# lucidrains/transfusion-pytorch

Hardware: AMD Instinct MI355X
Metric: train samples/sec, dim512 d8 seq1024 text+latent (higher is better)
Workload: dtype bf16; 1 GPU; BASELINE config 2: Transfusion dim=512 depth=8 heads=8 dim_head=64 num_text_tokens=256 dim_latent=384; per-GPU batch 64 x seq 1024 (32 x [24 text tokens + (4,384) latent] per sample); step = pack + fwd + bwd + clip(0.5) + Adam(3e-4) (one GPU: no gradient exchange); global_batch=64, seq_len=1024, parallelism=dp1

## Files before the change

include/tfx.h:

```cpp
#ifndef TFX_H
#define TFX_H
#include <stdint.h>
#ifdef __cplusplus
extern "C" {
#endif

#ifndef TFX_BF16_DEFINED
typedef uint16_t tfx_bf16;
#endif

enum { TFX_EPI_BF16 = 0, TFX_EPI_F32 = 1, TFX_EPI_SILU = 2, TFX_EPI_RESID = 3, TFX_EPI_GEGLU = 4, TFX_EPI_GEGLU_BWD = 5, TFX_EPI_QKV_NORM_ROPE = 6 };

typedef struct {
  const tfx_bf16* A; int32_t lda;
  const tfx_bf16* A2; int32_t lda2; int32_t K1;
  const tfx_bf16* B; int32_t ldb;
  int32_t M, N, K;
  int32_t epi;
  void* C; int32_t ldc;
  void* C2; int32_t ldc2;
  const float* bias;
  const tfx_bf16* R; int32_t ldr; int32_t resid_mapped;
  const int32_t* rowmap;
  const int32_t* a_rowmap;
  const tfx_bf16* aux; int32_t ldaux;
  int32_t qk_heads;
  const float* qk_gamma_q; const float* qk_gamma_k;
  const int32_t* qk_rot_pos; const float* qk_cos; const float* qk_sin;
  float qk_q_scale, qk_norm_scale;
  float* qk_plan; float qk_softcap;
  tfx_bf16* qk_cache; int32_t qk_ld_cache; const int32_t* qk_cache_pos;
  const void* prefetch; int64_t prefetch_bytes;
} tfx_gemm_nt_args;
int tfx_gemm_nt(const tfx_gemm_nt_args* a, void* stream);
int tfx_gemm_nt_plan(const tfx_gemm_nt_args* a, int32_t* kind, int32_t* grid);

int tfx_mfma_peak_probe(const void* ops, float* out, int32_t iters, int32_t blocks, void* stream);

typedef struct {
  const tfx_bf16* A; int32_t lda; int32_t a_cols;
  const tfx_bf16* B; int32_t ldb; int32_t b_cols;
  int32_t M, N, K;
  float* C; int32_t ldc;
  const int32_t* rowmap;
  int32_t k_valid;
  int32_t splits;
  int32_t accumulate;
  float alpha;
  const int32_t* a_rowmap;
  const int32_t* b_rowmap;
  float* colsum;
  int32_t k_group;
  const void* group_next;
} tfx_gemm_tn_args;
int tfx_gemm_tn(const tfx_gemm_tn_args* a, void* stream);
int tfx_gemm_tn_plan(const tfx_gemm_tn_args* a, int32_t* kind, int32_t* tiles, int32_t* splits, int32_t* grid);

typedef struct {
  const tfx_bf16 *q, *k, *v; int32_t ld_q, ld_k, ld_v;
  const tfx_bf16* gate; int32_t ld_gate;
  const int32_t* kv_end;
  const int32_t* q_start;
  tfx_bf16* out; int32_t ld_out;
  float* lse;
  int32_t b, h, n;
  float softcap;
  int32_t n_kv;
  const tfx_bf16* dout; int32_t ld_dout;
  tfx_bf16* do_eff; int32_t ld_do;
  float* delta;
  tfx_bf16* dgate; int32_t ld_dgate;
  tfx_bf16 *dq, *dk, *dv; int32_t ld_dq, ld_dk, ld_dv;
  int32_t order;
  const float* sc_plan;
  const int32_t* q_row0; const int32_t* q_cnt;
  const tfx_bf16* nr_qkv; int32_t nr_ld_qkv;
  tfx_bf16* nr_dqkv; int32_t nr_ld_dqkv;
  const float* nr_gamma_q; const float* nr_gamma_k;
  const int32_t* nr_rot_pos; const float* nr_cos; const float* nr_sin;
  float nr_q_scale, nr_norm_scale;
  float* nr_dgamma_q; float* nr_dgamma_k;
  int32_t laser;
} tfx_attn_args;
int tfx_attn_fwd(const tfx_attn_args* a, void* stream);
int tfx_attn_bwd(const tfx_attn_args* a, void* stream);

int tfx_decode_attn(const tfx_attn_args* a, void* stream);

typedef struct {
  int32_t T, H;
  const tfx_bf16* v; int32_t ld_v;
  tfx_bf16* vl; int32_t ld_vl;
  const int32_t* rowmap;
  float c;
// ... 278 lines not shown
```

transfusion_pytorch_amd/csrc/attention.hip:

```cpp
#include "tfx_kernels.h"
#include "attn_asm_clobbers.inc"

namespace tfx {

constexpr int DH = 64;
constexpr int LDT = 72;

struct TileRegs { u32x4 r[2]; };
TFX_DEV void tile_gload(TileRegs& tr, const bf16* base, int ld, int row0, int nrows) {
#pragma unroll
  for (int i = 0; i < 2; i++) {
    int c = threadIdx.x + 256 * i;
    int row = min(row0 + (c >> 3), nrows - 1);
    tr.r[i] = *(const u32x4*)(base + (size_t)row * ld + (c & 7) * 8);
  }
}
TFX_DEV void tile_sstore(const TileRegs& tr, bf16* lds) {
#pragma unroll
  for (int i = 0; i < 2; i++) {
    int c = threadIdx.x + 256 * i;
    *(u32x4*)(lds + (c >> 3) * LDT + (c & 7) * 8) = tr.r[i];
  }
}
TFX_DEV bf16x8 lds_rowfrag(const bf16* lds, int r0, int ks) {
// ... 482 lines not shown
  if (vid >= T * p.h) return;
  const unsigned t = vid / (unsigned)p.h; const int h = (int)(vid - t * p.h);
  const bf16x8 d8 = *(const bf16x8*)(p.dout + (size_t)t * p.ld_dout + h * DH + sub * 8);
  const bf16x8 o8 = *(const bf16x8*)(p.out + (size_t)t * p.ld_out + h * DH + sub * 8);
  const float g = sigmoidf_(bf2f(p.gate[(size_t)t * p.ld_gate + h]));
  if (p.laser) {
    const float rg = __builtin_amdgcn_rcpf(fmaxf(g, 1e-30f));
    float dg = 0.f, ds = 0.f; bf16x8 e8;
#pragma unroll
    for (int e = 0; e < 8; e++) {
      const float d = bf2f(d8[e]), og = bf2f(o8[e]);
      dg += d * og; ds += d;
      e8[e] = f2bf(d * g * __expf(-og * rg));
    }
    *(bf16x8*)(p.do_eff + (size_t)t * p.ld_do + h * DH + sub * 8) = e8;
    dg = group8_sum(dg); ds = group8_sum(ds);
    if (sub == 0) {
      const unsigned bb = t / (unsigned)p.n, i = t - bb * p.n;
      p.delta[((size_t)bb * p.h + h) * p.n + i] = ds * g;
      p.dgate[(size_t)t * p.ld_dgate + h] = f2bf(dg * (1.f - g));
    }
    return;
  }
  float dl = 0.f; bf16x8 e8;
#pragma unroll
  for (int e = 0; e < 8; e++) { float d = bf2f(d8[e]); dl += d * bf2f(o8[e]); e8[e] = f2bf(d * g); }
  *(bf16x8*)(p.do_eff + (size_t)t * p.ld_do + h * DH + sub * 8) = e8;
  dl = group8_sum(dl);
  if (sub == 0) {
    const unsigned bb = t / (unsigned)p.n, i = t - bb * p.n;
    p.delta[((size_t)bb * p.h + h) * p.n + i] = dl;
    p.dgate[(size_t)t * p.ld_dgate + h] = f2bf(dl * (1.f - g));
  }
}

__global__ __launch_bounds__(256, 2) void attn_bwd_dq_kernel(tfx_attn_args p) {
  __shared__ __attribute__((aligned(16))) bf16 Ks[64 * LDT];
  __shared__ __attribute__((aligned(16))) bf16 Vs[64 * LDT];
  const int l = threadIdx.x & 63, w = threadIdx.x >> 6, hi = l >> 5;
  const int n = p.n;
  const BlockId bi = decode_block(p.order, (n + 127) / 128, true);
  const int h = bi.h, b = bi.b, q0 = bi.tile * 128;
  const size_t tok0 = (size_t)b * n;
  const bf16* qb = p.q + tok0 * p.ld_q + h * DH;
  const bf16* kb_ = p.k + tok0 * p.ld_k + h * DH;
  const bf16* vb = p.v + tok0 * p.ld_v + h * DH;
  const bf16* dob = p.do_eff + tok0 * p.ld_do + h * DH;
  const int qrow = q0 + w * 32 + (l & 31);
  const int qc = min(qrow, n - 1);
  const int kve = p.kv_end[tok0 + qc];
  const int kv_limit = p.kv_end[tok0 + min(q0 + 127, n - 1)];
  const int nt = (kv_limit + 63) / 64;
  const float lse2 = p.lse[((size_t)b * p.h + h) * n + qc] * LOG2E;
  float dlt;
  const int kve_min = wave_min_i(kve);
// ... 464 lines not shown
      for (int e = 0; e < 8; e++) pg[e] = 0.f;
      wave_block_store_nr<1>(st, kv, p, tok0 + k0 + w * 32, (p.h + h) * DH, rows, pg);
      wave_block_store(st, vv, p.dv + (tok0 + k0 + w * 32) * p.ld_dv + h * DH, p.ld_dv, rows);
      nr_flush_dgamma(pg, sg, p.nr_dgamma_k);
    } else {
      wave_block_store(st, kv, p.dk + (tok0 + k0 + w * 32) * p.ld_dk + h * DH, p.ld_dk, rows);
      wave_block_store(st, vv, p.dv + (tok0 + k0 + w * 32) * p.ld_dv + h * DH, p.ld_dv, rows);
    }
  }
}

static dim3 attn_grid(const tfx_attn_args& q) { return dim3(q.h, q.b, (q.n + 127) / 128); }
int attn_fwd(const tfx_attn_args& p, hipStream_t s) {
  if (p.n <= 0 || p.b <= 0 || p.h <= 0) return -1;
  if ((p.ld_q | p.ld_k | p.ld_v | p.ld_out) & 7) return -2;
  if (!(p.softcap > 0.f) || p.softcap * LOG2E > 96.f) return -3;
  tfx_attn_args q = p; q.order = 1;
  static int use_asm = -1;
  if (use_asm < 0) { const char* e = getenv("TFX_ATTN_ASM"); use_asm = (e && e[0] == '1') ? 1 : 0; }
  if (use_asm && p.n_kv == 0 && !p.q_cnt && !p.q_row0 && p.sc_plan) hipLaunchKernelGGL(attn_fwd_pipe_kernel<true>, attn_grid(q), dim3(256), 0, s, q);
  else hipLaunchKernelGGL(attn_fwd_pipe_kernel<false>, attn_grid(q), dim3(256), 0, s, q);
  return (int)hipGetLastError();
}
int attn_bwd(const tfx_attn_args& p, hipStream_t s) {
  if (p.n <= 0 || p.b <= 0 || p.h <= 0) return -1;
  if ((p.ld_q | p.ld_k | p.ld_v | p.ld_out | p.ld_dout | p.ld_do | p.ld_dq | p.ld_dk | p.ld_dv) & 7) return -2;
  if (!(p.softcap > 0.f) || p.softcap * LOG2E > 96.f) return -3;
  long long nthreads = (long long)p.b * p.n * p.h * 8;
  if (nthreads >= (1ll << 31)) return -4;
  if (p.nr_qkv) {
    if (!p.nr_dqkv || !p.nr_gamma_q || !p.nr_gamma_k || !p.nr_rot_pos || !p.nr_cos || !p.nr_sin || !p.nr_dgamma_q || !p.nr_dgamma_k) return -5;
    if (((p.nr_ld_qkv | p.nr_ld_dqkv) & 7) || (((uintptr_t)p.nr_qkv | (uintptr_t)p.nr_dqkv) & 15)) return -5;
  }
  tfx_attn_args q = p; q.order = 1;
  static int pipe = -1;
  if (pipe < 0) { const char* e = getenv("TFX_ATTN_BWD_PIPE"); pipe = (e && e[0] == '0') ? 0 : 1; }
  hipLaunchKernelGGL(attn_bwd_prep_kernel, dim3((unsigned)((nthreads + 255) / 256)), dim3(256), 0, s, q);
  hipLaunchKernelGGL(attn_bwd_dkv_kernel, attn_grid(q), dim3(256), 0, s, q);
  if (pipe) hipLaunchKernelGGL(attn_bwd_dq_pipe_kernel, attn_grid(q), dim3(256), 0, s, q);
  else hipLaunchKernelGGL(attn_bwd_dq_kernel, attn_grid(q), dim3(256), 0, s, q);
  return (int)hipGetLastError();
}

}
```

transfusion_pytorch_amd/csrc/gemm.hip:

```cpp
#include "tfx_common.h"
#include "tfx_kernels.h"
#include <type_traits>
#include <cmath>
#include <cstring>
#include <vector>
#include <algorithm>
#include <mutex>

namespace tfx {

constexpr int BM = 128, BN = 128, BK = 64;

template <int EPI> struct Epilogue;

TFX_DEV void store_bf16x4(bf16* dst, f32x4 v) {
  bf16x4 o; o[0] = f2bf(v[0]); o[1] = f2bf(v[1]); o[2] = f2bf(v[2]); o[3] = f2bf(v[3]);
  *(bf16x4*)dst = o;
}

TFX_DEV f32x4 add_bias(const GemmNT& p, int n, f32x4 v) {
  if (p.bias) { f32x4 b = *(const f32x4*)(p.bias + n); v += b; }
  return v;
}

// ... 275 lines not shown
    }
    if (i + 1 < NI) load_r(i + 1);
    bf16* s = st + (i & 1) * 2048;
#pragma unroll
    for (int j = 0; j < 2; j++)
#pragma unroll
      for (int g = 0; g < 4; g++) {
        const int col = j * 32 + 8 * g + 4 * hi;
        const bf16x4 rv = *(const bf16x4*)(sr + r * 64 + (((col >> 3) ^ ((r >> 1) & 7)) << 3) + (col & 7));
        f32x4 v;
#pragma unroll
        for (int e = 0; e < 4; e++) v[e] = acc[i][j][4 * g + e] + bias[j][g][e] + bf2f(rv[e]);
        stage_put4(s, r, col, v);
      }
    bf16x8 v[4];
#pragma unroll
    for (int q = 0; q < 4; q++) {
      const int row = q * 8 + (l >> 3);
      v[q] = *(const bf16x8*)(s + row * 64 + ((ch ^ ((row >> 1) & 7)) << 3));
    }
#pragma unroll
    for (int q = 0; q < 4; q++)
      if (col_ok && mo[i][q] >= 0) *(bf16x8*)((bf16*)p.C + (size_t)mo[i][q] * p.ldc + n_w + ch * 8) = v[q];
  }
}
TFX_DEV void stage_put4_32(bf16* st, int row, int col, f32x4 v) {
  bf16x4 o; o[0] = f2bf(v[0]); o[1] = f2bf(v[1]); o[2] = f2bf(v[2]); o[3] = f2bf(v[3]);
  *(bf16x4*)(st + row * 32 + (((col >> 3) ^ ((row >> 2) & 3)) << 3) + (col & 7)) = o;
}
constexpr int GTAB_N = 4096;
TFX_DEV float gelu_grid(const float* gtab, float g) {
  const float x = g * 128.f;
  const float xr = __builtin_amdgcn_fmed3f(__builtin_rintf(x), -1024.f, 1023.f);
  const float d = x - xr;
  const f32x4 c = *(const f32x4*)(gtab + 4 * ((int)xr + 1024));
  return fmaf(fmaf(c[2], d, c[1]), d, c[0]);
}
TFX_DEV GegluUVH geglu_uvh_grid(const float* gtab, float a, float g) {
  const float x = g * 128.f;
  const float xr = __builtin_amdgcn_fmed3f(__builtin_rintf(x), -1024.f, 1023.f);
  const float d = x - xr;
  const f32x4 c = *(const f32x4*)(gtab + 4 * ((int)xr + 1024));
  const float t = fmaf(c[2], d, c[1]);
  GegluUVH r; r.u = fmaf(t, d, c[0]);
  r.h = a * r.u;
  r.v = (a * 128.f) * fmaf(c[2], d, t);
// ... 283 lines not shown
  }
}
template <int EPI> TFX_DEV bool can_stage(const GemmNT& p) {
  bool ok = ((p.ldc | p.N) & 7) == 0 && (((uintptr_t)p.C) & 15) == 0;
  if constexpr (EPI == EPI_GEGLU) ok = ok && (p.ldc2 & 7) == 0 && (((uintptr_t)p.C2) & 15) == 0;
  if constexpr (EPI == EPI_GEGLU_BWD) ok = ok && (p.ldaux & 7) == 0 && (((uintptr_t)p.aux) & 15) == 0 && p.N >= 64;
  if constexpr (EPI == EPI_RESID) ok = ok && (p.ldr & 7) == 0 && (((uintptr_t)p.R) & 15) == 0 && p.N >= 8;
  return ok;
}
template <int EPI, int NI>
TFX_DEV void nt_epilogue(const GemmNT& p, f32x16 (&acc)[NI][2], int m_w, int n_w, bf16* st, const float* gtab = nullptr, bool use_tab = false, int lane = -1) {
  if constexpr (EPI == EPI_BF16) {
    if (can_stage<EPI>(p)) {
      if (!p.rowmap && !p.bias) staged_epilogue_bf16<NI, true>(p, acc, m_w, n_w, st, lane);
      else staged_epilogue_bf16<NI, false>(p, acc, m_w, n_w, st, lane);
      return;
    }
  } else if constexpr (EPI == EPI_F32) {
    if (((p.ldc | p.N) & 3) == 0 && (((uintptr_t)p.C) & 15) == 0) { staged_epilogue_f32<NI>(p, acc, m_w, n_w, st); return; }
  } else if constexpr (EPI == EPI_GEGLU || EPI == EPI_GEGLU_BWD) {
    if (can_stage<EPI>(p)) { staged_epilogue_geglu<EPI, NI>(p, acc, m_w, n_w, st, gtab, use_tab); return; }
  } else if constexpr (EPI == EPI_RESID) {
    if (can_stage<EPI>(p)) { staged_epilogue_resid<NI>(p, acc, m_w, n_w, st); return; }
  }
  if constexpr (EPI == EPI_QKNR) staged_epilogue_qknr<NI>(p, acc, m_w, n_w, st);
  else fast_epilogue<EPI, NI>(p, acc, m_w, n_w, lane);
}


template <int EPI>
__global__ __launch_bounds__(256, 2) void gemm_nt_kernel(GemmNT p) {
  extern __shared__ __attribute__((aligned(16))) char smem_raw[];
  bf16* As = (bf16*)smem_raw;
  bf16* Bs = As + 2 * BM * BK;

  const int t = threadIdx.x, l = t & 63, w = t >> 6;
  const int wm = w >> 1, wn = w & 1, hi = l >> 5;
  const int ntn = (p.N + BN - 1) / BN;
  const int bid = xcd_remap(blockIdx.x, gridDim.x);
  const int m0 = (bid / ntn) * BM, n0 = (bid % ntn) * BN;
  const int nk = p.K / BK;

  int srow[4], skc[4];
  const bf16 *ga[4], *ga2[4], *gb[4];
#pragma unroll
  for (int i = 0; i < 4; i++) {
// ... 658 lines not shown
    const int k0 = kt * BK;
    const bool second = p.A2 && k0 >= p.K1;
    glds16_asm(second ? gA2[h][j] + (k0 - p.K1) : gA[h][j] + k0, lds + ((kt & 1) * 4 + h) * HALF + (w * 16 + j * 8) * BK);
  };
  auto issueB1 = [&](int kt, int h, int j) { glds16_asm(gB[h][j] + kt * BK, lds + ((kt & 1) * 4 + 2 + h) * HALF + (w * 16 + j * 8) * BK); };
  const int ra = wr * 64 + (l & 31), rb = wc * 32 + (l & 31);
  auto ldA = [&](int kt, int h, int il, int ks) {
    const int r = ra + il * 32;
    return *(const bf16x8*)(lds + ((kt & 1) * 4 + h) * HALF + r * BK + (((ks * 2 + hi) ^ ((r >> 1) & 7)) << 3));
  };
  auto ldB = [&](int kt, int h, int ks) {
    return *(const bf16x8*)(lds + ((kt & 1) * 4 + 2 + h) * HALF + rb * BK + (((ks * 2 + hi) ^ ((rb >> 1) & 7)) << 3));
  };

  f32x16 acc[4][2];
#pragma unroll
  for (int i = 0; i < 4; i++)
#pragma unroll
    for (int j = 0; j < 2; j++)
#pragma unroll
      for (int r = 0; r < 16; r++) acc[i][j][r] = 0.f;

#ifdef TFX_PP_TIMING
  unsigned long long* stamps = (unsigned long long*)(EPI == EPI_GEGLU_BWD ? (const void*)p.R : (const void*)p.aux) + (size_t)blockIdx.x * 8;
#define PP_STAMP(i) { if (t == 0) stamps[i] = __builtin_readcyclecounter(); }
#else
#define PP_STAMP(i)
#endif
  PP_STAMP(0)
  asm volatile("s_waitcnt vmcnt(0)" ::: "memory");
  if constexpr (EPI == EPI_QKNR) {
    if (p.qk_plan && blockIdx.x == 0 && w == 0) softcap_plan_write(p.qk_gamma_q, p.qk_gamma_k, p.qk_norm_scale, p.qk_q_scale, p.qk_softcap, p.qk_plan);
  }
  const float* gtab_lds = (const float*)(smem_raw + 8 * HALF * 2);
  if constexpr (EPI == EPI_GEGLU) {
    if (gtab) {
#pragma unroll
      for (int j = 0; j < 4; j++) glds16_asm((const bf16*)gtab + (size_t)(w * 4 + j) * 512 + l * 8, (const bf16*)gtab_lds + (w * 4 + j) * 512);
    }
  }
  issueA(0, 0); issueB(0, 0); issueA(0, 1); issueB(0, 1);
  if (nk > 1) {
    issueA(1, 0); issueB(1, 0);
    asm volatile("s_waitcnt vmcnt(4)" ::: "memory");
  } else {
    asm volatile("s_waitcnt vmcnt(0)" ::: "memory");
  }
// ... 587 lines not shown
    auto phi = [](double g) { return 0.39894228040143267794 * exp(-0.5 * g * g); };
    const double st = 1.0 / 128.0;
    for (int i = 0; i < 2048; i++) {
      const double g = (i - 1024) * st;
      h[4 * i] = (float)(g * Phi(g));
      h[4 * i + 1] = (float)((Phi(g) + g * phi(g)) * st);
      h[4 * i + 2] = (float)(0.5 * phi(g) * (2.0 - g * g) * st * st);
      h[4 * i + 3] = 0.f;
    }
    float* d = nullptr;
    if (hipMalloc(&d, h.size() * 4) == hipSuccess && hipMemcpy(d, h.data(), h.size() * 4, hipMemcpyHostToDevice) == hipSuccess) tab[dev] = d;
  }
  return tab[dev];
}
struct NtPlan { int kind, grid; };
static bool nt_ow_takes(const GemmNT& p);
static bool nt_owp_takes(const GemmNT& p);
static NtPlan nt_plan(const GemmNT& p) {
  const int grid = ((p.M + BM - 1) / BM) * ((p.N + BN - 1) / BN);
  const int t256 = ((p.M + BM2 - 1) / BM2) * ((p.N + BN2 - 1) / BN2);
  const bool dma = use_glds() && (p.N & 3) == 0;
  const int grid_sd = ((p.M + 63) / 64) * ((p.N + 63) / 64);
  const int grid_sk = ((p.M + SK_BM - 1) / SK_BM) * ((p.N + SK_BN - 1) / SK_BN);
  if (dma && p.M <= 1024 && p.K % SD_BK == 0 && p.K >= 8 * SD_BK && grid_sd <= 256) return {NT_DECODE, grid_sd};
  if (dma && (p.M <= 512 || (p.M <= 1024 && grid_sk <= 256))) return {NT_SKINNY, grid_sk};
  static int pp_min = -1;
  if (pp_min < 0) { const char* e = getenv("TFX_NT_PP_MIN"); pp_min = e ? atoi(e) : 512; }
  if (dma && t256 >= pp_min) return {!nt_ow_takes(p) ? NT_PP : nt_owp_takes(p) ? NT_OWP : NT_OW, t256};
  if (dma && grid <= 256 && p.K >= 4 * BK) return {NT_MID, grid};
  return {dma ? NT_GLDS : NT_FALLBACK, grid};
}

constexpr int PP_STAGGER = 12000;
template <int EPI> static void launch_pp(const GemmNT& p, int grid, hipStream_t s) {
  static uint32_t attr_pp = 0;
  const float* gtab = EPI == EPI_GEGLU ? gelu_table() : nullptr;
  const int smem2 = 2 * (BM2 * BK + BN2 * BK) * 2 + (gtab ? GTAB_N * 8 : 0);
  ensure_smem_attr((const void*)gemm_nt_pp_kernel<EPI>, 2 * (BM2 * BK + BN2 * BK) * 2 + GTAB_N * 8, attr_pp);
  hipLaunchKernelGGL(gemm_nt_pp_kernel<EPI>, dim3(grid), dim3(512), smem2, s, p, PP_STAGGER, gtab);
}
static int nt_ow_mode() {
  static int ow = -1;
  if (ow < 0) { const char* e = getenv("TFX_NT_OW"); ow = e ? atoi(e) : 1; }
  return ow;
}
static bool nt_ow_takes(const GemmNT& p) {
  const int ow = nt_ow_mode();
  if (ow == 0 || p.a_rowmap || p.A2) return false;
  if (!(p.epi == EPI_BF16 || (p.epi == EPI_F32 && p.K >= 1024))) return false;
  if ((((uintptr_t)p.A | (uintptr_t)p.B) & 15) != 0) return false;
// ... 73 lines not shown
  return !p.rowmap && !p.a_rowmap && !p.bias && ((p.ldc | p.ldc2 | p.N) & 7) == 0 && (((uintptr_t)p.C | (uintptr_t)p.C2) & 15) == 0 && 2 * hd <= p.N && p.ldc2 >= 2 * hd;
}
static int gemm_nt_qknr(const GemmNT& p, hipStream_t s) {
  if (p.qk_heads <= 0 || !p.C2 || !p.qk_gamma_q || !p.qk_gamma_k || !p.qk_rot_pos || !p.qk_cos || !p.qk_sin) return -5;
  if (qknr_fusable(p)) {
    const NtPlan pl = nt_plan(p);
    if (pl.kind == NT_PP) { launch_pp<EPI_QKNR>(p, pl.grid, s); return (int)hipGetLastError(); }
    static uint32_t attr_sd = 0;
    const int smem_sd = 4 * SD_ST * SD_SLOT * 2;
    ensure_smem_attr((const void*)gemm_nt_decode_kernel<EPI_QKNR>, smem_sd, attr_sd);
    hipLaunchKernelGGL(gemm_nt_decode_kernel<EPI_QKNR>, dim3(pl.grid + prefetch_blocks(p)), dim3(256), smem_sd, s, p, pl.grid);
    return (int)hipGetLastError();
  }
  GemmNT q = p; q.epi = EPI_BF16; q.C2 = nullptr;
  const int rc = launch_nt<EPI_BF16>(q, s);
  if (rc) return rc;
  tfx_qk_norm_rope_args a;
  memset(&a, 0, sizeof(a));
  a.T = p.M; a.H = p.qk_heads; a.qkv = (const tfx_bf16*)p.C; a.ld_qkv = p.ldc; a.qk = (tfx_bf16*)p.C2; a.ld_qk = p.ldc2;
  a.gamma_q = p.qk_gamma_q; a.gamma_k = p.qk_gamma_k; a.rot_pos = p.qk_rot_pos; a.cos_tab = p.qk_cos; a.sin_tab = p.qk_sin;
  a.q_scale = p.qk_q_scale; a.norm_scale = p.qk_norm_scale; a.sc_plan = p.qk_plan; a.softcap = p.qk_softcap;
  a.cache = p.qk_cache; a.ld_cache = p.qk_ld_cache; a.cache_pos = p.qk_cache_pos;
  return tfx_qk_norm_rope_fwd(&a, (void*)s);
}

int gemm_nt(const GemmNT& p, hipStream_t s) {
  if (p.K % BK != 0 || (p.A2 && p.K1 % BK != 0) || p.M <= 0 || p.N <= 0) return -1;
  if ((p.lda | p.ldb) & 7) return -2;
  switch (p.epi) {
    case EPI_BF16: return launch_nt<EPI_BF16>(p, s);
    case EPI_F32: return launch_nt<EPI_F32>(p, s);
    case EPI_SILU: return launch_nt<EPI_SILU>(p, s);
    case EPI_RESID: return launch_nt<EPI_RESID>(p, s);
    case EPI_GEGLU: return (p.N % 64) ? -3 : launch_nt<EPI_GEGLU>(p, s);
    case EPI_GEGLU_BWD: return (p.N % 64) ? -3 : launch_nt<EPI_GEGLU_BWD>(p, s);
    case EPI_QKNR: return gemm_nt_qknr(p, s);
  }
  return -4;
}

template <bool SUM, int FA, int FB, int WN, int WK, int NST> static void launch_tn_wide(const GemmTN& q, int grid, hipStream_t s) {
  constexpr int smem = NST * (FA * WN + FB * WK) / 4 * MW_ROWS * 128 * 2;
  static uint32_t attr = 0;
  ensure_smem_attr((const void*)gemm_tn_wide_kernel<SUM, FA, FB, WN, WK, NST>, smem, attr);
  hipLaunchKernelGGL((gemm_tn_wide_kernel<SUM, FA, FB, WN, WK, NST>), dim3(grid), dim3(64 * WN * WK), smem, s, q);
}

struct TnPlan { int kind, tiles, splits, grid; };
static int tn_ow_mode();
static bool tn_ow_operands_ok(const GemmTN& q);
static TnPlan tn_plan(const GemmTN& q) {
#ifdef TFX_TN_TIMING
  const bool dma_ok = true;
#else
  const bool dma_ok = use_glds() && q.M % TN_BMK == 0 && !q.a_rowmap && !q.b_rowmap && q.a_cols >= 8 && q.b_cols >= 8;
#endif
  const int t44 = ((q.N + 255) / 256) * ((q.K + 255) / 256), t22 = ((q.N + 127) / 128) * ((q.K + 127) / 128);
  TnPlan pl;
  pl.kind = !dma_ok ? -1 : (t44 >= 8 ? 2 : 0);
// ... 129 lines not shown
```

transfusion_pytorch_amd/csrc/tfx_common.h:

```cpp
#pragma once
#include <hip/hip_runtime.h>
#include <stdint.h>
#include <mutex>

typedef __bf16 bf16;
typedef __attribute__((ext_vector_type(8))) __bf16 bf16x8;
typedef __attribute__((ext_vector_type(4))) __bf16 bf16x4;
typedef __attribute__((ext_vector_type(2))) __bf16 bf16x2;
typedef __attribute__((ext_vector_type(16))) float f32x16;
typedef __attribute__((ext_vector_type(4))) float f32x4;
typedef __attribute__((ext_vector_type(2))) float f32x2_t;
typedef __attribute__((ext_vector_type(4))) short s16x4;
typedef __attribute__((ext_vector_type(4))) uint32_t u32x4;
typedef __attribute__((ext_vector_type(2))) uint32_t u32x2;

#define TFX_DEV __device__ __forceinline__

TFX_DEV float bf2f(bf16 v) { return (float)v; }
TFX_DEV bf16 f2bf(float v) { return (bf16)v; }

#ifndef TFX_BPERMUTE_REDUCE
#define TFX_DPP_STEP(OP, V, CTRL, ROWMASK, IDENT)                                                                     \
  V = OP(V, __builtin_bit_cast(float, __builtin_amdgcn_update_dpp(__builtin_bit_cast(int, (float)(IDENT)),            \
                                                                    __builtin_bit_cast(int, V), CTRL, ROWMASK, 0xf, false)))
// ... 102 lines not shown
  asm volatile("s_mov_b32 m0, %1\n\ts_nop 0\n\tglobal_load_lds_dwordx4 %0, off" ::"v"(g), "s"(lds_addr) : "memory");
}

TFX_DEV float gelu_cdf(float g, float& E) {
  E = __expf(-0.5f * g * g);
  const float t = __builtin_amdgcn_rcpf(fmaf(0.3275911f * 0.70710678118654752440f, fabsf(g), 1.f));
  const float poly = t * fmaf(t, fmaf(t, fmaf(t, fmaf(t, 1.061405429f, -1.453152027f), 1.421413741f), -0.284496736f), 0.254829592f);
  const float half_erf = 0.5f - 0.5f * poly * E;
  return 0.5f + __builtin_copysignf(half_erf, g);
}
TFX_DEV float gelu_erf(float x) { float E; return x * gelu_cdf(x, E); }
struct GegluUVH { float u, v, h; };
TFX_DEV GegluUVH geglu_uvh(float a, float g) {
  float E; const float cdf = gelu_cdf(g, E);
  GegluUVH r; r.u = g * cdf; r.h = a * r.u;
  r.v = a * fmaf(g * 0.39894228040143267794f, E, cdf);
  return r;
}
TFX_DEV float gelu_erf_grad(float x) {
  return 0.5f * (1.f + erff(x * 0.70710678118654752440f)) + x * 0.39894228040143267794f * __expf(-0.5f * x * x);
}
TFX_DEV float sigmoidf_(float x) { return __builtin_amdgcn_rcpf(1.f + __expf(-x)); }

inline std::mutex& smem_attr_mutex() { static std::mutex mu; return mu; }
inline void ensure_smem_attr(const void* fn, int bytes, uint32_t& done_mask) {
  int dev = 0;
  if (hipGetDevice(&dev) != hipSuccess) dev = 0;
  const uint32_t bit = 1u << (dev & 31);
  std::lock_guard<std::mutex> lock(smem_attr_mutex());
  if (!(done_mask & bit)) { (void)hipFuncSetAttribute(fn, hipFuncAttributeMaxDynamicSharedMemorySize, bytes); done_mask |= bit; }
}
```

transfusion_pytorch_amd/csrc/tfx_kernels.h:

```cpp
#pragma once
#include "tfx_common.h"
#define TFX_BF16_DEFINED
typedef __bf16 tfx_bf16;
#include "../../include/tfx.h"

namespace tfx {
using GemmNT = tfx_gemm_nt_args;
using GemmTN = tfx_gemm_tn_args;
enum { EPI_BF16 = TFX_EPI_BF16, EPI_F32 = TFX_EPI_F32, EPI_SILU = TFX_EPI_SILU, EPI_RESID = TFX_EPI_RESID,
       EPI_GEGLU = TFX_EPI_GEGLU, EPI_GEGLU_BWD = TFX_EPI_GEGLU_BWD, EPI_QKNR = TFX_EPI_QKV_NORM_ROPE };
int gemm_nt(const GemmNT& p, hipStream_t s);
int gemm_tn(const GemmTN& p, hipStream_t s);
int gemm_nt_plan(const GemmNT& p, int* kind, int* grid);
int gemm_tn_plan(const GemmTN& p, int* kind, int* tiles, int* splits, int* grid);
int attn_fwd(const tfx_attn_args& p, hipStream_t s);
int attn_bwd(const tfx_attn_args& p, hipStream_t s);
}
```

transfusion_pytorch_amd/engine.py:

```python
from __future__ import annotations

import ctypes
import os
import weakref

import torch

from . import capi
from .params import ModelDims, ParamStore, pad_to

BF16 = torch.bfloat16
E = capi.ENUMS


def _p(t, *idx):
    for i in idx:
        t = t[i]
    return t.data_ptr()


def skip_sources(md: ModelDims):
    stack, src = [], {}
    for i in range(md.depth):
        layer = i + 1
# ... 215 lines not shown
                self.vlc = side.get(key)
                if self.vlc is None:
                    self.vlc = e(D, cache.shape[1] * cache.shape[2], hd)
                    side[key] = self.vlc
        self.fwd, self.bwd = LaunchList(), LaunchList()
        self.noise_args = {}
        self.loaded_structure = None
        self._seg_args = []
        self.seg_start = z(max(T, 1), dtype=torch.int32); self.seg_len = z(max(T, 1), dtype=torch.int32)
        self.pull = training and D <= 32 and md.dim <= 1024
        if self.pull:
            self.arsave = [e(T, i + 2, 4, dtype=torch.float32) for i in range(D)]
            self.arerr = e(D, T, d)
        self._build_forward()
        if training:
            self.dH = e(D + 1, T, d)
            self.gx = {i: e(T, d) for i in range(D) if md.has_skip(i)}; self.du = e(T, d)
            env = os.environ.get('TFX_SIDE_STREAM')
            self.side = D <= 30 and (env == '1' or (env is None and md.dim <= 1024))
            nb = 2 if self.side else 1
            self.dy_f = [e(T, d) for _ in range(nb)]; self.dy_a = [e(T, d) for _ in range(nb)] if self.side else self.dy_f
            self.dskip = {j: e(T, d) for j in set(skip_sources(md).values())}
            self.dqkvg_p = [z(T, ldq) for _ in range(nb)]; self.dog = e(T, hd); self.do_eff = e(T, hd)
            self.dqk = e(T, 2 * hd) if os.environ.get('TFX_ATTN_QKNR', '1') == '0' else None
            self.delta = e(b, md.heads, n, dtype=torch.float32)
            self.dag_p = [e(T, 2 * dip) for _ in range(nb)]; self.dembed = e(T, d); self.gfin = e(T, d); self.dx0 = e(T, d)
            self.dtables = z(I1, nt3, dtype=torch.float32); self.dtab_bf = e(I1, nt3)
            self.dcond = e(I1, 4 * d); self.dpre = e(I1, 4 * d)
            self.onehot = e(T, md.vp)
            self._build_backward()

    def _nt(self, lst, algo_n=None, algo_k=None, **kw):
        a = capi.make_args('tfx_gemm_nt_args', **kw)
        a._algo_flops = 2.0 * kw['M'] * (algo_n or kw['N']) * (algo_k or kw['K'])
        lst.append(('tfx_gemm_nt', a))

    def _tn(self, lst, M, N, K, **kw):
        splits = 0
        kw.setdefault('k_valid', K)
        algo_n = kw.pop('algo_n', None)
        side = kw.pop('side', False)
        a = capi.make_args('tfx_gemm_tn_args', M=M, N=N, K=K, splits=splits, accumulate=1, alpha=1.0, **kw)
        a._algo_flops = 2.0 * M * (algo_n or N) * kw['k_valid']
        lst.append(Side(('tfx_gemm_tn', a)) if side else ('tfx_gemm_tn', a))

    def _tn_group(self, lst, M, problems, side=False):
# ... 261 lines not shown
        self.clean_mode = mode
        for t, a in self._clean_launch.items():
            lt = self.lat[t]
            a[1] = lt['q'].data_ptr() if mode == 'model' else lt['x'].data_ptr()
            a[2] = None if mode == 'model' else self.noise_args[t].eps

    def _attn_kw(self, i, bwd=False):
        md, hd, ldq = self.md, self.md.hdk, self.md.ldq
        li, lkv = self._li(i), self._lkv(i)
        kw = dict(q=self.qkr[lkv], k=_p(self.qkr, lkv) + 2 * hd, v=_p(self.qkvg, lkv) + 2 * 2 * hd, ld_q=2 * hd, ld_k=2 * hd, ld_v=ldq,
                  gate=_p(self.qkvg, lkv) + 2 * 3 * hd, ld_gate=ldq, kv_end=self.kv_end, q_start=self.q_start, out=self.og[li], ld_out=hd,
                  lse=self.lse[li], b=self.units[0] if self.units else self.b, h=md.heads, n=self.units[1] if self.units else self.n, softcap=50.0)
        if self.units:
            kw.update(q_row0=self.unit_row0, q_cnt=self.unit_cnt)
        if self.sc_plan is not None:
            kw['sc_plan'] = self.sc_plan[i]
        if self.cache is not None:
            ck = self.cache[i]
            kw.update(k=ck.data_ptr(), v=ck.data_ptr() + 2 * hd, ld_k=2 * hd, ld_v=2 * hd, n_kv=int(ck.shape[1]))
        if md.laser:
            kw.update(v=self.vl[li] if self.cache is None else self.vlc[i], ld_v=hd, laser=1)
        if bwd:
            dqkvg = self.dqkvg_p[i % len(self.dqkvg_p)]
            kw.update(dout=self.dog, ld_dout=hd, do_eff=self.do_eff, ld_do=hd, delta=self.delta,
                      dgate=dqkvg.data_ptr() + 2 * 3 * hd, ld_dgate=ldq, dq=self.dqk if self.dqk is not None else 0,
                      dk=self.dqk.data_ptr() + 2 * hd if self.dqk is not None else 0,
                      dv=dqkvg.data_ptr() + 2 * 2 * hd, ld_dq=2 * hd, ld_dk=2 * hd, ld_dv=ldq)
        return kw

    def set_rope_tables(self, cos_tab, sin_tab):
        if self.cos_tab is not None and (self.cos_tab.data_ptr() != cos_tab.data_ptr() or self.sin_tab.data_ptr() != sin_tab.data_ptr()):
            self.fwd.invalidate_graphs()
        self.cos_tab, self.sin_tab = cos_tab, sin_tab
        for a in getattr(self, '_rope_args', []):
            a.cos_tab, a.sin_tab = cos_tab.data_ptr(), sin_tab.data_ptr()
        for a in getattr(self, '_rope_nt_args', []):
            a.qk_cos, a.qk_sin = cos_tab.data_ptr(), sin_tab.data_ptr()
        for a in getattr(self, '_rope_attn_args', []):
            a.nr_cos, a.nr_sin = cos_tab.data_ptr(), sin_tab.data_ptr()

    def set_segments(self, seg_start, seg_len):
        n_seg = int(seg_start.numel())
        self.seg_start[:n_seg].copy_(seg_start); self.seg_len[:n_seg].copy_(seg_len)
        for a in self._seg_args:
            a.n_seg = n_seg

    def set_rows(self, R_true: dict):
# ... 146 lines not shown
                g2 = self.dskip[i + 1] if (i + 1) in pushed else None
                self._k(L, 'tfx_attnres_bwd', 'tfx_attnres_args', T=T, d=d, L=i + 2, hiddens=self.hid, stride_h=T * d,
                        gamma=pp(f'{p}.3.norm_keys.gamma'), pq=pp(f'{p}.3.pseudo_queries'), g=g, g2=capi.ptr(g2), dhiddens=self.dH, stride_dh=T * d,
                        first=1 if i == D - 1 else 0, dgamma=gp(f'{p}.3.norm_keys.gamma'), dpq=gp(f'{p}.3.pseudo_queries'))
                L.append(('tfx_adaln_post_bwd', a_postf))
            self._nt(L, algo_n=di, A=dy_f, lda=d, B=S[f'ff2_t{i}'], ldb=d, M=T, N=dip, K=d, epi=E['TFX_EPI_GEGLU_BWD'], C=dag, ldc=2 * dip,
                     aux=self.ag[i], ldaux=2 * dip)
            sync('tfx_fork', 2 * i)
            ff_grp = [(d, di, dict(A=dy_f, lda=d, a_cols=d, B=self.hm[i], ldb=dip, b_cols=dip, C=gp(f'{p}.2.fn.net.3.weight'), ldc=di)),
                      (2 * dip, d, dict(algo_n=2 * di, A=dag, lda=2 * dip, a_cols=2 * dip, B=self.uf[i], ldb=d, b_cols=d, rowmap=gmap,
                                        C=gp(f'{p}.2.fn.net.0.weight'), ldc=d, colsum=gp(f'{p}.2.fn.net.0.bias')))]
            self._tn_group(L, T, ff_grp, side=side)
            self._nt(L, algo_k=2 * di, A=dag, lda=2 * dip, B=S[f'ff1_t{i}'], ldb=2 * dip, M=T, N=d, K=2 * dip, epi=E['TFX_EPI_BF16'], C=self.du, ldc=d)
            a_pref = capi.make_args('tfx_adaln_pre_args', T=T, d=d, x=self.xb[i], tok_inst=self.tok_inst, table=tf, ld_table=nt3,
                                    gamma_text=pp(f'{p}.2.layernorm_gamma'), mean=_p(self.stats, 2, i), rstd=_p(self.stats, 3, i), du=self.du, dx=G,
                                    dtable=dtf, dgamma_text=gp(f'{p}.2.layernorm_gamma'), seg_start=self.seg_start, seg_len=self.seg_len, n_seg=0)
            a_posta = capi.make_args('tfx_adaln_post_args', T=T, d=d, y=self.ya[i], tok_inst=self.tok_inst, table=ta, ld_table=nt3,
                                     layerscale=pp(f'{p}.1.layerscale'), g=G, dy=dy_a, dtable=dta, dlayerscale=gp(f'{p}.1.layerscale'),
                                     seg_start=self.seg_start, seg_len=self.seg_len, n_seg=0)
            self._seg_args += [a_pref, a_posta]
            self._keep = getattr(self, '_keep', []) + [a_pref, a_posta]
            self._raw(L, lib.tfx_adaln_pre_post_bwd, ctypes.addressof(a_pref), ctypes.addressof(a_posta))
            self._hbm(L, 6)
            self._nt(L, algo_n=md.hd, A=dy_a, lda=d, B=S[f'out_t{i}'], ldb=d, M=T, N=hd, K=d, epi=E['TFX_EPI_BF16'], C=self.dog, ldc=hd)
            gam = (lambda nm: S[f'g{nm}{i}']) if md.dim_head != 64 else (lambda nm: pp(f'{p}.1.fn.{nm}_norm.gamma'))
            if os.environ.get('TFX_ATTN_QKNR', '1') != '0':
                self._k(L, 'tfx_attn_bwd', 'tfx_attn_args', **self._attn_kw(i, bwd=True), nr_qkv=self.qkvg[i], nr_ld_qkv=ldq, nr_dqkv=dqkvg, nr_ld_dqkv=ldq,
                        nr_gamma_q=gam('q'), nr_gamma_k=gam('k'), nr_rot_pos=self.rot_pos, nr_cos=0, nr_sin=0, nr_q_scale=md.dim_head ** -0.5,
                        nr_norm_scale=md.dim_head ** 0.5, nr_dgamma_q=gp(f'{p}.1.fn.q_norm.gamma'), nr_dgamma_k=gp(f'{p}.1.fn.k_norm.gamma'))
                self._rope_attn_args = getattr(self, '_rope_attn_args', []) + [L[-1][1]]
            else:
                self._k(L, 'tfx_attn_bwd', 'tfx_attn_args', **self._attn_kw(i, bwd=True))
                self._k(L, 'tfx_qk_norm_rope_bwd', 'tfx_qk_norm_rope_args', T=T, H=H, qkv=self.qkvg[i], ld_qkv=ldq, gamma_q=gam('q'),
                        gamma_k=gam('k'), rot_pos=self.rot_pos, cos_tab=0, sin_tab=0, q_scale=md.dim_head ** -0.5, norm_scale=md.dim_head ** 0.5,
                        dqk=self.dqk, ld_dqk=2 * hd, dqkv=dqkvg, ld_dqkv=ldq, dgamma_q=gp(f'{p}.1.fn.q_norm.gamma'), dgamma_k=gp(f'{p}.1.fn.k_norm.gamma'))
                self._rope_args = getattr(self, '_rope_args', []) + [L[-1][1]]
                L.meta = L.meta or {}
                L.meta[len(L) - 1] = ('hbm', 3 * 2 * T * hd * 2)
            if md.laser:
                dv = dqkvg.data_ptr() + 2 * 2 * hd
                self._k(L, 'tfx_laser_v_bwd', 'tfx_laser_v_args', T=T, H=H, v=_p(self.qkvg, i) + 2 * 2 * hd, ld_v=ldq, c=md.laser,
                        dvl=dv, ld_dvl=ldq, dv=dv, ld_dv=ldq)
                L.meta = L.meta or {}
                L.meta[len(L) - 1] = ('hbm', 3 * T * hd * 2)
            self._nt(L, algo_k=md.nq, A=dqkvg, lda=ldq, B=S[f'qkvg_t{i}'], ldb=ldq, M=T, N=d, K=ldq, epi=E['TFX_EPI_BF16'], C=self.du, ldc=d)
            self._k(L, 'tfx_adaln_pre_bwd', 'tfx_adaln_pre_args', T=T, d=d, x=x_a, tok_inst=self.tok_inst, table=ta, ld_table=nt3,
                    gamma_text=pp(f'{p}.1.layernorm_gamma'), mean=_p(self.stats, 0, i), rstd=_p(self.stats, 1, i), du=self.du, dx=G,
# ... 161 lines not shown
```

Before: 2569 samples/s.

## Fuse attention-backward prep into the output-projection backward GEMM epilogue

Adds a GEMM NT epilogue (EPI_ATTN_PREP) that computes do_eff, delta and dgate directly from the accumulator for the dO = dy @ W_out product. It loads the forward output and gate alongside the tile, and the attention backward skips its separate prep kernel via prep_done. This removes one kernel launch and a bf16 write and read of the intermediate dO tensor per layer. In exchange the epilogue does more work and forces the PP GEMM path. A fallback (plain GEMM into scratch, then the prep kernel) covers non-fusable cases.

```diff
diff --git a/include/tfx.h b/include/tfx.h
--- a/include/tfx.h
+++ b/include/tfx.h
@@ -9,7 +9,7 @@
 typedef uint16_t tfx_bf16;
 #endif
 
-enum { TFX_EPI_BF16 = 0, TFX_EPI_F32 = 1, TFX_EPI_SILU = 2, TFX_EPI_RESID = 3, TFX_EPI_GEGLU = 4, TFX_EPI_GEGLU_BWD = 5, TFX_EPI_QKV_NORM_ROPE = 6 };
+enum { TFX_EPI_BF16 = 0, TFX_EPI_F32 = 1, TFX_EPI_SILU = 2, TFX_EPI_RESID = 3, TFX_EPI_GEGLU = 4, TFX_EPI_GEGLU_BWD = 5, TFX_EPI_QKV_NORM_ROPE = 6, TFX_EPI_ATTN_PREP = 7 };
 
 typedef struct {
   const tfx_bf16* A; int32_t lda;
@@ -31,6 +31,11 @@
   float* qk_plan; float qk_softcap;
   tfx_bf16* qk_cache; int32_t qk_ld_cache; const int32_t* qk_cache_pos;
   const void* prefetch; int64_t prefetch_bytes;
+  const tfx_bf16* ap_gate; int32_t ap_ld_gate;
+  float* ap_delta;
+  tfx_bf16* ap_dgate; int32_t ap_ld_dgate;
+  int32_t ap_n, ap_h;
+  tfx_bf16* ap_scratch; int32_t ap_ld_scratch;
 } tfx_gemm_nt_args;
 int tfx_gemm_nt(const tfx_gemm_nt_args* a, void* stream);
 int tfx_gemm_nt_plan(const tfx_gemm_nt_args* a, int32_t* kind, int32_t* grid);
@@ -70,6 +75,7 @@
   tfx_bf16* do_eff; int32_t ld_do;
   float* delta;
   tfx_bf16* dgate; int32_t ld_dgate;
+  int32_t prep_done;
   tfx_bf16 *dq, *dk, *dv; int32_t ld_dq, ld_dk, ld_dv;
   int32_t order;
   const float* sc_plan;
diff --git a/transfusion_pytorch_amd/csrc/attention.hip b/transfusion_pytorch_amd/csrc/attention.hip
--- a/transfusion_pytorch_amd/csrc/attention.hip
+++ b/transfusion_pytorch_amd/csrc/attention.hip
@@ -528,15 +528,14 @@
     }
     return;
   }
-  float dl = 0.f; bf16x8 e8;
-#pragma unroll
-  for (int e = 0; e < 8; e++) { float d = bf2f(d8[e]); dl += d * bf2f(o8[e]); e8[e] = f2bf(d * g); }
+  bf16x8 e8;
+  float dl = attn_prep_chunk(d8, o8, g, e8);
   *(bf16x8*)(p.do_eff + (size_t)t * p.ld_do + h * DH + sub * 8) = e8;
   dl = group8_sum(dl);
   if (sub == 0) {
     const unsigned bb = t / (unsigned)p.n, i = t - bb * p.n;
     p.delta[((size_t)bb * p.h + h) * p.n + i] = dl;
-    p.dgate[(size_t)t * p.ld_dgate + h] = f2bf(dl * (1.f - g));
+    p.dgate[(size_t)t * p.ld_dgate + h] = attn_prep_dgate(dl, g);
   }
 }
 
@@ -1047,9 +1046,17 @@
   else hipLaunchKernelGGL(attn_fwd_pipe_kernel<false>, attn_grid(q), dim3(256), 0, s, q);
   return (int)hipGetLastError();
 }
+int attn_bwd_prep(const tfx_attn_args& p, hipStream_t s) {
+  if (p.n <= 0 || p.b <= 0 || p.h <= 0) return -1;
+  if ((p.ld_out | p.ld_dout | p.ld_do) & 7) return -2;
+  const long long nthreads = (long long)p.b * p.n * p.h * 8;
+  if (nthreads >= (1ll << 31)) return -4;
+  hipLaunchKernelGGL(attn_bwd_prep_kernel, dim3((unsigned)((nthreads + 255) / 256)), dim3(256), 0, s, p);
+  return (int)hipGetLastError();
+}
 int attn_bwd(const tfx_attn_args& p, hipStream_t s) {
   if (p.n <= 0 || p.b <= 0 || p.h <= 0) return -1;
-  if ((p.ld_q | p.ld_k | p.ld_v | p.ld_out | p.ld_dout | p.ld_do | p.ld_dq | p.ld_dk | p.ld_dv) & 7) return -2;
+  if ((p.ld_q | p.ld_k | p.ld_v | p.ld_out | (p.prep_done ? 0 : p.ld_dout) | p.ld_do | p.ld_dq | p.ld_dk | p.ld_dv) & 7) return -2;
   if (!(p.softcap > 0.f) || p.softcap * LOG2E > 96.f) return -3;
   long long nthreads = (long long)p.b * p.n * p.h * 8;
   if (nthreads >= (1ll << 31)) return -4;
@@ -1060,7 +1067,7 @@
   tfx_attn_args q = p; q.order = 1;
   static int pipe = -1;
   if (pipe < 0) { const char* e = getenv("TFX_ATTN_BWD_PIPE"); pipe = (e && e[0] == '0') ? 0 : 1; }
-  hipLaunchKernelGGL(attn_bwd_prep_kernel, dim3((unsigned)((nthreads + 255) / 256)), dim3(256), 0, s, q);
+  if (!p.prep_done) { const int rc = attn_bwd_prep(q, s); if (rc) return rc; }
   hipLaunchKernelGGL(attn_bwd_dkv_kernel, attn_grid(q), dim3(256), 0, s, q);
   if (pipe) hipLaunchKernelGGL(attn_bwd_dq_pipe_kernel, attn_grid(q), dim3(256), 0, s, q);
   else hipLaunchKernelGGL(attn_bwd_dq_kernel, attn_grid(q), dim3(256), 0, s, q);
diff --git a/transfusion_pytorch_amd/csrc/gemm.hip b/transfusion_pytorch_amd/csrc/gemm.hip
--- a/transfusion_pytorch_amd/csrc/gemm.hip
+++ b/transfusion_pytorch_amd/csrc/gemm.hip
@@ -321,6 +321,64 @@
 #pragma unroll
     for (int q = 0; q < 4; q++)
       if (col_ok && mo[i][q] >= 0) *(bf16x8*)((bf16*)p.C + (size_t)mo[i][q] * p.ldc + n_w + ch * 8) = v[q];
+  }
+}
+template <int NI>
+TFX_DEV void staged_epilogue_attn_prep(const GemmNT& p, f32x16 (&acc)[NI][2], int m_w, int n_w, bf16* st) {
+  if (n_w >= p.N || m_w >= p.M) return;
+  const int l = threadIdx.x & 63, hi = l >> 5, r = l & 31, ch = l & 7, lr = l >> 3;
+  const int h = n_w >> 6;
+  const unsigned n = (unsigned)p.ap_n, q8 = 8u / n, r8 = 8u % n;
+  unsigned bb = (unsigned)(m_w + lr) / n, pos = (unsigned)(m_w + lr) - bb * n;
+  const bf16* ogp = p.aux + n_w + ch * 8;
+  const bf16* gtp = p.ap_gate + h;
+  bf16x8 og[4]; bf16 gl[4];
+  auto load_side = [&](int i) {
+#pragma unroll
+    for (int q = 0; q < 4; q++) {
+      const int m = min(m_w + i * 32 + q * 8 + lr, p.M - 1);
+      og[q] = *(const bf16x8*)(ogp + (size_t)m * p.ldaux);
+      gl[q] = gtp[(size_t)m * p.ap_ld_gate];
+    }
+  };
+  load_side(0);
+#pragma unroll
+  for (int i = 0; i < NI; i++) {
+    bf16* s = st + (i & 1) * 2048;
+#pragma unroll
+    for (int j = 0; j < 2; j++)
+#pragma unroll
+      for (int g = 0; g < 4; g++) {
+        f32x4 v;
+#pragma unroll
+        for (int e = 0; e < 4; e++) v[e] = acc[i][j][4 * g + e];
+        stage_put4(s, r, j * 32 + 8 * g + 4 * hi, v);
+      }
+    bf16x8 v[4];
+#pragma unroll
+    for (int q = 0; q < 4; q++) {
+      const int row = q * 8 + lr;
+      v[q] = *(const bf16x8*)(s + row * 64 + ((ch ^ ((row >> 1) & 7)) << 3));
+    }
+    float dsel = 0.f, gsel = 0.f; unsigned isel = 0; int msel = p.M;
+#pragma unroll
+    for (int q = 0; q < 4; q++) {
+      const float g = sigmoidf_(bf2f(gl[q]));
+      bf16x8 e8;
+      const float dl = group8_sum(attn_prep_chunk(v[q], og[q], g, e8));
+      v[q] = e8;
+      if (ch == q) { dsel = dl; gsel = g; isel = (bb * (unsigned)p.ap_h + h) * n + pos; msel = m_w + i * 32 + q * 8 + lr; }
+      pos += r8; bb += q8;
+      if (pos >= n) { pos -= n; bb++; }
+    }
+    if (i + 1 < NI) load_side(i + 1);
+#pragma unroll
+    for (int q = 0; q < 4; q++)
+      if (m_w + i * 32 + q * 8 + lr < p.M) *(bf16x8*)((bf16*)p.C + (size_t)(m_w + i * 32 + q * 8 + lr) * p.ldc + n_w + ch * 8) = v[q];
+    if (msel < p.M) {
+      p.ap_delta[isel] = dsel;
+      p.ap_dgate[(size_t)msel * p.ap_ld_dgate + h] = attn_prep_dgate(dsel, gsel);
+    }
   }
 }
 TFX_DEV void stage_put4_32(bf16* st, int row, int col, f32x4 v) {
@@ -650,6 +708,9 @@
     if (can_stage<EPI>(p)) { staged_epilogue_geglu<EPI, NI>(p, acc, m_w, n_w, st, gtab, use_tab); return; }
   } else if constexpr (EPI == EPI_RESID) {
     if (can_stage<EPI>(p)) { staged_epilogue_resid<NI>(p, acc, m_w, n_w, st); return; }
+  } else if constexpr (EPI == EPI_ATTN_PREP) {
+    staged_epilogue_attn_prep<NI>(p, acc, m_w, n_w, st);
+    return;
   }
   if constexpr (EPI == EPI_QKNR) staged_epilogue_qknr<NI>(p, acc, m_w, n_w, st);
   else fast_epilogue<EPI, NI>(p, acc, m_w, n_w, lane);
@@ -1354,7 +1415,7 @@
       for (int r = 0; r < 16; r++) acc[i][j][r] = 0.f;
 
 #ifdef TFX_PP_TIMING
-  unsigned long long* stamps = (unsigned long long*)(EPI == EPI_GEGLU_BWD ? (const void*)p.R : (const void*)p.aux) + (size_t)blockIdx.x * 8;
+  unsigned long long* stamps = (unsigned long long*)(EPI == EPI_GEGLU_BWD || EPI == EPI_ATTN_PREP ? (const void*)p.R : (const void*)p.aux) + (size_t)blockIdx.x * 8;
 #define PP_STAMP(i) { if (t == 0) stamps[i] = __builtin_readcyclecounter(); }
 #else
 #define PP_STAMP(i)
@@ -1988,10 +2049,11 @@
   const bool dma = use_glds() && (p.N & 3) == 0;
   const int grid_sd = ((p.M + 63) / 64) * ((p.N + 63) / 64);
   const int grid_sk = ((p.M + SK_BM - 1) / SK_BM) * ((p.N + SK_BN - 1) / SK_BN);
+  static int pp_min = -1;
+  if (pp_min < 0) { const char* e = getenv("TFX_NT_PP_MIN"); pp_min = e ? atoi(e) : 512; }
+  if (dma && p.epi == EPI_ATTN_PREP && t256 >= pp_min) return {NT_PP, t256};
   if (dma && p.M <= 1024 && p.K % SD_BK == 0 && p.K >= 8 * SD_BK && grid_sd <= 256) return {NT_DECODE, grid_sd};
   if (dma && (p.M <= 512 || (p.M <= 1024 && grid_sk <= 256))) return {NT_SKINNY, grid_sk};
-  static int pp_min = -1;
-  if (pp_min < 0) { const char* e = getenv("TFX_NT_PP_MIN"); pp_min = e ? atoi(e) : 512; }
   if (dma && t256 >= pp_min) return {!nt_ow_takes(p) ? NT_PP : nt_owp_takes(p) ? NT_OWP : NT_OW, t256};
   if (dma && grid <= 256 && p.K >= 4 * BK) return {NT_MID, grid};
   return {dma ? NT_GLDS : NT_FALLBACK, grid};
@@ -2111,6 +2173,27 @@
   a.q_scale = p.qk_q_scale; a.norm_scale = p.qk_norm_scale; a.sc_plan = p.qk_plan; a.softcap = p.qk_softcap;
   a.cache = p.qk_cache; a.ld_cache = p.qk_ld_cache; a.cache_pos = p.qk_cache_pos;
   return tfx_qk_norm_rope_fwd(&a, (void*)s);
+}
+
+static bool attn_prep_fusable(const GemmNT& p) {
+  if (nt_plan(p).kind != NT_PP) return false;
+  return !p.rowmap && !p.a_rowmap && !p.bias && ((p.ldc | p.ldaux) & 7) == 0 && (((uintptr_t)p.C | (uintptr_t)p.aux) & 15) == 0;
+}
+static int gemm_nt_attn_prep(const GemmNT& p, hipStream_t s) {
+  if (p.ap_h <= 0 || p.ap_n <= 0 || p.N != 64 * p.ap_h || p.M % p.ap_n != 0 || p.rowmap) return -6;
+  if (!p.C || !p.aux || !p.ap_gate || !p.ap_delta || !p.ap_dgate) return -6;
+  if ((long long)p.M * p.ap_h * 8 >= (1ll << 31)) return -6;
+  if (attn_prep_fusable(p)) { launch_pp<EPI_ATTN_PREP>(p, nt_plan(p).grid, s); return (int)hipGetLastError(); }
+  if (!p.ap_scratch || (p.ap_ld_scratch & 7)) return -6;
+  GemmNT q = p; q.epi = EPI_BF16; q.C = p.ap_scratch; q.ldc = p.ap_ld_scratch;
+  const int rc = launch_nt<EPI_BF16>(q, s);
+  if (rc) return rc;
+  tfx_attn_args a;
+  memset(&a, 0, sizeof(a));
+  a.b = p.M / p.ap_n; a.n = p.ap_n; a.h = p.ap_h;
+  a.dout = p.ap_scratch; a.ld_dout = p.ap_ld_scratch; a.out = (tfx_bf16*)p.aux; a.ld_out = p.ldaux; a.gate = p.ap_gate; a.ld_gate = p.ap_ld_gate;
+  a.do_eff = (tfx_bf16*)p.C; a.ld_do = p.ldc; a.delta = p.ap_delta; a.dgate = p.ap_dgate; a.ld_dgate = p.ap_ld_dgate;
+  return attn_bwd_prep(a, s);
 }
 
 int gemm_nt(const GemmNT& p, hipStream_t s) {
@@ -2124,6 +2207,7 @@
     case EPI_GEGLU: return (p.N % 64) ? -3 : launch_nt<EPI_GEGLU>(p, s);
     case EPI_GEGLU_BWD: return (p.N % 64) ? -3 : launch_nt<EPI_GEGLU_BWD>(p, s);
     case EPI_QKNR: return gemm_nt_qknr(p, s);
+    case EPI_ATTN_PREP: return gemm_nt_attn_prep(p, s);
   }
   return -4;
 }
diff --git a/transfusion_pytorch_amd/csrc/tfx_common.h b/transfusion_pytorch_amd/csrc/tfx_common.h
--- a/transfusion_pytorch_amd/csrc/tfx_common.h
+++ b/transfusion_pytorch_amd/csrc/tfx_common.h
@@ -148,6 +148,18 @@
 }
 TFX_DEV float sigmoidf_(float x) { return __builtin_amdgcn_rcpf(1.f + __expf(-x)); }
 
+TFX_DEV float attn_prep_chunk(const bf16x8 d8, const bf16x8 o8, float g, bf16x8& e8) {
+#pragma clang fp contract(off)
+  float dl = 0.f;
+#pragma unroll
+  for (int e = 0; e < 8; e++) { const float d = bf2f(d8[e]); dl = __builtin_fmaf(d, bf2f(o8[e]), dl); e8[e] = f2bf(d * g); }
+  return dl;
+}
+TFX_DEV bf16 attn_prep_dgate(float delta, float g) {
+#pragma clang fp contract(off)
+  return f2bf(delta * (1.f - g));
+}
+
 inline std::mutex& smem_attr_mutex() { static std::mutex mu; return mu; }
 inline void ensure_smem_attr(const void* fn, int bytes, uint32_t& done_mask) {
   int dev = 0;
diff --git a/transfusion_pytorch_amd/csrc/tfx_kernels.h b/transfusion_pytorch_amd/csrc/tfx_kernels.h
--- a/transfusion_pytorch_amd/csrc/tfx_kernels.h
+++ b/transfusion_pytorch_amd/csrc/tfx_kernels.h
@@ -8,11 +8,12 @@
 using GemmNT = tfx_gemm_nt_args;
 using GemmTN = tfx_gemm_tn_args;
 enum { EPI_BF16 = TFX_EPI_BF16, EPI_F32 = TFX_EPI_F32, EPI_SILU = TFX_EPI_SILU, EPI_RESID = TFX_EPI_RESID,
-       EPI_GEGLU = TFX_EPI_GEGLU, EPI_GEGLU_BWD = TFX_EPI_GEGLU_BWD, EPI_QKNR = TFX_EPI_QKV_NORM_ROPE };
+       EPI_GEGLU = TFX_EPI_GEGLU, EPI_GEGLU_BWD = TFX_EPI_GEGLU_BWD, EPI_QKNR = TFX_EPI_QKV_NORM_ROPE, EPI_ATTN_PREP = TFX_EPI_ATTN_PREP };
 int gemm_nt(const GemmNT& p, hipStream_t s);
 int gemm_tn(const GemmTN& p, hipStream_t s);
 int gemm_nt_plan(const GemmNT& p, int* kind, int* grid);
 int gemm_tn_plan(const GemmTN& p, int* kind, int* tiles, int* splits, int* grid);
 int attn_fwd(const tfx_attn_args& p, hipStream_t s);
 int attn_bwd(const tfx_attn_args& p, hipStream_t s);
+int attn_bwd_prep(const tfx_attn_args& p, hipStream_t s);
 }
diff --git a/transfusion_pytorch_amd/engine.py b/transfusion_pytorch_amd/engine.py
--- a/transfusion_pytorch_amd/engine.py
+++ b/transfusion_pytorch_amd/engine.py
@@ -261,6 +261,7 @@
             self.dy_f = [e(T, d) for _ in range(nb)]; self.dy_a = [e(T, d) for _ in range(nb)] if self.side else self.dy_f
             self.dskip = {j: e(T, d) for j in set(skip_sources(md).values())}
             self.dqkvg_p = [z(T, ldq) for _ in range(nb)]; self.dog = e(T, hd); self.do_eff = e(T, hd)
+            self.prep_fused = md.dim_head == 64 and not md.laser and os.environ.get('TFX_ATTN_PREP_FUSED', '1') != '0'
             self.dqk = e(T, 2 * hd) if os.environ.get('TFX_ATTN_QKNR', '1') == '0' else None
             self.delta = e(b, md.heads, n, dtype=torch.float32)
             self.dag_p = [e(T, 2 * dip) for _ in range(nb)]; self.dembed = e(T, d); self.gfin = e(T, d); self.dx0 = e(T, d)
@@ -568,7 +569,7 @@
             kw.update(v=self.vl[li] if self.cache is None else self.vlc[i], ld_v=hd, laser=1)
         if bwd:
             dqkvg = self.dqkvg_p[i % len(self.dqkvg_p)]
-            kw.update(dout=self.dog, ld_dout=hd, do_eff=self.do_eff, ld_do=hd, delta=self.delta,
+            kw.update(**(dict(dout=0, ld_dout=0, prep_done=1) if self.prep_fused else dict(dout=self.dog, ld_dout=hd)), do_eff=self.do_eff, ld_do=hd, delta=self.delta,
                       dgate=dqkvg.data_ptr() + 2 * 3 * hd, ld_dgate=ldq, dq=self.dqk if self.dqk is not None else 0,
                       dk=self.dqk.data_ptr() + 2 * hd if self.dqk is not None else 0,
                       dv=dqkvg.data_ptr() + 2 * 2 * hd, ld_dq=2 * hd, ld_dk=2 * hd, ld_dv=ldq)
@@ -761,7 +762,12 @@
             self._keep = getattr(self, '_keep', []) + [a_pref, a_posta]
             self._raw(L, lib.tfx_adaln_pre_post_bwd, ctypes.addressof(a_pref), ctypes.addressof(a_posta))
             self._hbm(L, 6)
-            self._nt(L, algo_n=md.hd, A=dy_a, lda=d, B=S[f'out_t{i}'], ldb=d, M=T, N=hd, K=d, epi=E['TFX_EPI_BF16'], C=self.dog, ldc=hd)
+            if self.prep_fused:
+                self._nt(L, algo_n=md.hd, A=dy_a, lda=d, B=S[f'out_t{i}'], ldb=d, M=T, N=hd, K=d, epi=E['TFX_EPI_ATTN_PREP'], C=self.do_eff, ldc=hd,
+                         aux=self.og[i], ldaux=hd, ap_gate=_p(self.qkvg, i) + 2 * 3 * hd, ap_ld_gate=ldq, ap_delta=self.delta,
+                         ap_dgate=dqkvg.data_ptr() + 2 * 3 * hd, ap_ld_dgate=ldq, ap_n=self.n, ap_h=md.heads, ap_scratch=self.dog, ap_ld_scratch=hd)
+            else:
+                self._nt(L, algo_n=md.hd, A=dy_a, lda=d, B=S[f'out_t{i}'], ldb=d, M=T, N=hd, K=d, epi=E['TFX_EPI_BF16'], C=self.dog, ldc=hd)
             gam = (lambda nm: S[f'g{nm}{i}']) if md.dim_head != 64 else (lambda nm: pp(f'{p}.1.fn.{nm}_norm.gamma'))
             if os.environ.get('TFX_ATTN_QKNR', '1') != '0':
                 self._k(L, 'tfx_attn_bwd', 'tfx_attn_args', **self._attn_kw(i, bwd=True), nr_qkv=self.qkvg[i], nr_ld_qkv=ldq, nr_dqkv=dqkvg, nr_ld_dqkv=ldq,
```

Result: no change. 2581 samples/s, median of 6 (+0.4%).
